# apache/incubator-predictionio

Measured on NVIDIA H100. Metric: ALS iterations/sec, higher is better.
Workload: dtype f32

## Files before the change

### incubator-predictionio_b200/csrc/als_kernels.cuh

```cuda
#pragma once
#include <cuda_runtime.h>
#include <stdint.h>

#include "als_lockstep.cuh"

namespace pio {

struct SolveParams {
  const long long* ptr;
  const int* idx;
  const float* val;
  const float* src;
  float* dst;
  const float* yty;
  const float* nreg;
  int* fail;
  float lambda;
  float alpha;
  int k;
  int row_begin;
  int row_end;
  int dst_row_offset;
  const unsigned* absmax;
  const long long* wl_beg;
// ... 501 lines not shown
    for (int o = lane; o < SLOT + KP; o += 32) {
      float s = 0.f;
      for (int q = p0; q < p1; ++q) s += p.partial[(size_t)q * (SLOT + KP) + o];
      slot[o] = s;
    }
    __syncwarp();
    chol_solve_warp<Cfg::WARP_CHOL ? KP : 16, Cfg::TB, Cfg::BLK, IMPLICIT>(
        slot, bv, p.yty, p.lambda * p.nreg[r], p.k, colbuf, dinv, p.dst + (size_t)(p.dst_row_offset + r) * KP, p.fail);
  }
}

constexpr int FIN128_WARPS = 6;
constexpr int FIN128_FLOATS = LsLayout<128>::STRIDE + 128 + 80;

template <bool IMPLICIT>
__global__ void __launch_bounds__(32 * FIN128_WARPS, 1)
als_finish_ls128_kernel(const SolveParams p, const int* __restrict__ row_part_ptr, int row0, int n_rows, int part0) {
  using LL = LsLayout<128>;
  constexpr int PF = LL::SIZE + 128;
  extern __shared__ __align__(16) float fsm128[];
  const int warp = threadIdx.x >> 5, lane = threadIdx.x & 31;
  float* slot = fsm128 + warp * FIN128_FLOATS;
  float* bv = slot + LL::STRIDE;
  float* colbuf = bv + 128;
#pragma unroll 1
  for (int base = blockIdx.x * FIN128_WARPS; base < n_rows; base += gridDim.x * FIN128_WARPS) {
    const int rr = base + warp;
    const bool have = rr < n_rows;
    const int r = row0 + (have ? rr : 0);
    if (have) {
      const int p0 = row_part_ptr[r] - part0, p1 = row_part_ptr[r + 1] - part0;
      for (int o = lane; o < PF / 4; o += 32) {
        float4 s = make_float4(0.f, 0.f, 0.f, 0.f);
        for (int q = p0; q < p1; ++q) {
          const float4 v = __ldg(reinterpret_cast<const float4*>(p.partial + (size_t)q * PF) + o);
          s.x += v.x; s.y += v.y; s.z += v.z; s.w += v.w;
        }
        if (o < LL::SIZE / 4) reinterpret_cast<float4*>(slot)[o] = s;
        else reinterpret_cast<float4*>(bv)[o - LL::SIZE / 4] = s;
      }
      if (IMPLICIT) {
        __syncwarp();
        ls_add_yty<128>(slot, p.yty);
      }
    }
    __syncthreads();
    if (have)
      chol_lockstep<128>(slot, bv, p.lambda * p.nreg[r], p.k, colbuf, p.dst + (size_t)(p.dst_row_offset + r) * 128, true,
                         p.fail);
    __syncthreads();
  }
}

constexpr int GRAM_THREADS = 256;
constexpr int GRAM_ROWS = 32;
constexpr int GRAM_GROUPS = 8;
struct GramMap {
  int cls[GRAM_GROUPS];
  int slot_of[GRAM_GROUPS];
};

template <int KP>
__global__ void __launch_bounds__(GRAM_THREADS)
gram_partial_kernel(const float* __restrict__ X, const int* __restrict__ p2i, int n_rows, double* __restrict__ partial,
                    int slot0, int bpg, const GramMap map) {
  constexpr int TM = KP / 16;
  __shared__ __align__(16) float tile[GRAM_ROWS * KP];
  const int tid = threadIdx.x, ty = tid / 16, tx = tid % 16;
  double acc[TM][TM];
#pragma unroll
  for (int i = 0; i < TM; ++i)
#pragma unroll
    for (int j = 0; j < TM; ++j) acc[i][j] = 0.0;
  const int lg = blockIdx.x / bpg, b = blockIdx.x % bpg, g = map.cls[lg];
  const int rem = n_rows % 16;
  const int T = 2 * (n_rows / 16) + (g < rem ? 1 : 0) + (15 - g < rem ? 1 : 0);
  const int per = (T + bpg - 1) / bpg;
  const int t0 = min(T, b * per);
  const int t1 = min(T, t0 + per);
  for (int base = t0; base < t1; base += GRAM_ROWS) {
    const int nr = min(GRAM_ROWS, t1 - base);
    for (int o = tid; o < GRAM_ROWS * KP / 4; o += GRAM_THREADS) {
      const int rr = o / (KP / 4);
      float4 v = make_float4(0.f, 0.f, 0.f, 0.f);
      if (rr < nr) {
        const int t = base + rr;
        const int pos = 16 * (t >> 1) + ((t & 1) ? 15 - g : g);
        v = reinterpret_cast<const float4*>(X + (size_t)__ldg(p2i + pos) * KP)[o % (KP / 4)];
      }
      reinterpret_cast<float4*>(tile)[o] = v;
    }
    __syncthreads();
#pragma unroll 4
    for (int rr = 0; rr < GRAM_ROWS; ++rr) {
      double a[TM], bb[TM];
#pragma unroll
      for (int i = 0; i < TM; ++i) {
        a[i] = (double)tile[rr * KP + ty * TM + i];
        bb[i] = (double)tile[rr * KP + tx * TM + i];
      }
#pragma unroll
      for (int i = 0; i < TM; ++i)
#pragma unroll
        for (int j = 0; j < TM; ++j) acc[i][j] = fma(a[i], bb[j], acc[i][j]);
    }
    __syncthreads();
  }
  double* out = partial + ((size_t)(slot0 + lg) * bpg + b) * KP * KP;
#pragma unroll
  for (int i = 0; i < TM; ++i)
#pragma unroll
    for (int j = 0; j < TM; ++j) out[(ty * TM + i) * KP + tx * TM + j] = acc[i][j];
}

__global__ void gram_group_kernel(const double* __restrict__ partial, int blocks_per_group, int n, int g0,
                                  double* __restrict__ gsum) {
  const int o = blockIdx.x * blockDim.x + threadIdx.x;
  const int g = g0 + blockIdx.y;
  if (o >= n) return;
  const double* p = partial + (size_t)g * blocks_per_group * n;
  double s = 0.0;
  for (int q = 0; q < blocks_per_group; ++q) s += p[(size_t)q * n + o];
  gsum[(size_t)g * n + o] = s;
}

__global__ void gram_reduce_kernel(const double* __restrict__ gsum, int n, float* __restrict__ out, const GramMap map) {
  const int o = blockIdx.x * blockDim.x + threadIdx.x;
  if (o >= n) return;
  double s = 0.0;
#pragma unroll
  for (int g = 0; g < GRAM_GROUPS; ++g) s += gsum[(size_t)map.slot_of[g] * n + o];
  out[o] = (float)s;
}

}
```

### incubator-predictionio_b200/csrc/pio_als.cu

```cuda
#include "../../include/pio_als.h"

#include <cuda_runtime.h>
#include <dlfcn.h>
#include <math.h>
#include <nccl.h>
#include <stdarg.h>
#include <stdio.h>
#include <stdlib.h>
#include <string.h>

#include <chrono>
#include <algorithm>
#include <array>
#include <deque>
#include <exception>
#include <map>
#include <memory>
#include <mutex>
#include <string>
#include <type_traits>
#include <vector>

#include "als_kernels.cuh"
#include "als_mma_kernel.cuh"
// ... 312 lines not shown
    int tz = h3 == 0 ? 64 : __ffsll((long long)h3) - 1;
    if (tz > 9) tz = 9;
    r[e] = (float)(1 + tz);
  } else {
    r[e] = (float)(1 + (int)(h3 % 5ull));
  }
}

struct Side {
  int n = 0;
  int R = 0;
  int n_internal = 0;
  int bits = 1;
  int* perm = nullptr;
  int* inv = nullptr;
  int* rpos = nullptr;
  int* p2i = nullptr;
  uint32_t* deg = nullptr;
  uint32_t* npos = nullptr;
  long long* ptr = nullptr;
  int* idx = nullptr;
  float* val = nullptr;
  long long nnz_local = 0;
  float* nreg = nullptr;
  float* F = nullptr;
  int* cand_ext = nullptr;
  int n_active = 0, n_heavy = 0;
  SidePlan plan;
  long long* part_beg = nullptr;
  long long* part_end = nullptr;
  int* row_part_ptr = nullptr;
  float* partial = nullptr;
  int n_parts = 0;
  std::vector<int> h_row_part_ptr;
};

enum EvKind { EV_SOLVE = 0, EV_GRAM = 1, EV_COMM = 2, EV_SOLVE_USER = 3, EV_NKIND = 4 };
struct EvPair {
  cudaEvent_t a, b;
  int kind;
};

}

using namespace pio;

struct pio_als_handle {
  pio_als_config cfg;
  int KP = 0;
  cudaStream_t stream = nullptr;
  Side U, I;
  float* yty = nullptr;
  double* gram_partial = nullptr;
  double* gram_gsum = nullptr;
  const Side* gram_side = nullptr;
  cudaEvent_t ev_gram = nullptr;
  int gram_blocks = 0;
  int* d_fail = nullptr;
  int* d_counts = nullptr;
  unsigned* d_absmax = nullptr;
  long long* d_timing = nullptr;
  float* d_dbg = nullptr;
  size_t dbg_rows = 0;
  SolveSwitches sw;
  cudaStream_t aux = nullptr, comm_st = nullptr;
  cudaEvent_t ev_start = nullptr, ev_heavy = nullptr, ev_piece[8] = {}, ev_comm = nullptr;
  bool pieces_done = false;
  bool trace_on = false;
  std::chrono::steady_clock::time_point t_prev;
  unsigned char* srv_dev = nullptr;
  size_t srv_dev_cap = 0;
  unsigned char* srv_host = nullptr;
  unsigned char* srv_host_dev = nullptr;
  size_t srv_host_cap = 0;
  unsigned* srv_counter = nullptr;
  unsigned srv_seq = 0;
  bool serve_fused = true;
  bool score_blocked = true;
  bool serve_trace = false;
  float* tc_out = nullptr;
  size_t tc_out_rows = 0;
  bool have_ratings = false, have_init = false, trained = false;
  ncclComm_t comm = nullptr;
  std::string err;
  pio_als_stats st{};
  double phase_ms[8] = {0, 0, 0, 0, 0, 0, 0, 0};
  std::deque<EvPair> ev_pool;
  size_t ev_used = 0;
  std::mutex mu;
  int sm_count = 0;
};

namespace pio {

static int vfail(std::string& sink, int code, const char* fmt, va_list ap) {
  char buf[512];
  vsnprintf(buf, sizeof buf, fmt, ap);
  sink = buf;
  return code;
}
static int fail(pio_als_handle* h, int code, const char* fmt, ...) {
  va_list ap;
  va_start(ap, fmt);
  const int rc = vfail(h ? h->err : g_create_error, code, fmt, ap);
  va_end(ap);
  return rc;
// ... 704 lines not shown
            tp.sp = p;
            tp.out = h->sw.tc_split ? h->tc_out : nullptr;
            tp.out_row0 = L.row_begin;
            rc = solve_launch(h, tc::Api::kernel(imp), L.grid, tc::Api::kThreads, tc::Api::kSmem, false, st, tp);
            break;
          default:
            rc = fp32();
        }
        break;
      case STAGE_TC_SOLVE:
        rc = solve_launch(h, tc::Api::solver(imp), L.grid, 32 * tc::Api::kSolveWarps, tc::Api::kSolveSmem, false, st, p,
                          (const float*)h->tc_out, L.row_begin);
        break;
    }
    if (rc) return rc;
    record_events((int)i + 1);
  }
  if (pair) {
    cudaStreamWaitEvent(h->stream, h->ev_heavy, 0);
    h->pieces_done = true;
  }
  return PIO_ALS_OK;
}

static int launch_solve(pio_als_handle* h, Side& dst, const Side& src) {
  switch (h->KP) {
    case 16: return launch_solve_cfg<Cfg16>(h, dst, src);
    case 32: return launch_solve_cfg<Cfg32>(h, dst, src);
    case 64: return launch_solve_cfg<Cfg64>(h, dst, src);
    default: return launch_solve_cfg<Cfg128>(h, dst, src);
  }
}

static bool gram_sharded(const pio_als_handle* h) { return h->cfg.world_size > 1 && GRAM_GROUPS % h->cfg.world_size == 0; }
static void gram_layout(const pio_als_handle* h, GramMap& m, int& my_groups, int& slot0) {
  const bool shard = gram_sharded(h);
  const int W = shard ? h->cfg.world_size : 1, me = shard ? h->cfg.world_rank : 0;
  my_groups = GRAM_GROUPS / W;
  slot0 = me * my_groups;
  int seen[GRAM_GROUPS] = {}, mine = 0;
  for (int g = 0; g < GRAM_GROUPS; ++g) {
    const int blk = g / W, pos = g % W;
    const int owner = (blk & 1) ? (W - 1 - pos) : pos;
    m.slot_of[g] = owner * my_groups + seen[owner]++;
    if (owner == me) m.cls[mine++] = g;
  }
  for (int lg = mine; lg < GRAM_GROUPS; ++lg) m.cls[lg] = 0;
}
static int gram_local(pio_als_handle* h, const Side& s) {
  GramMap m;
  int my_groups, slot0;
  gram_layout(h, m, my_groups, slot0);
  const int bpg = h->gram_blocks / GRAM_GROUPS, n = h->KP * h->KP, grid = my_groups * bpg;
  switch (h->KP) {
    case 16: gram_partial_kernel<16><<<grid, GRAM_THREADS, 0, h->stream>>>(s.F, s.p2i, s.n, h->gram_partial, slot0, bpg, m); break;
    case 32: gram_partial_kernel<32><<<grid, GRAM_THREADS, 0, h->stream>>>(s.F, s.p2i, s.n, h->gram_partial, slot0, bpg, m); break;
    case 64: gram_partial_kernel<64><<<grid, GRAM_THREADS, 0, h->stream>>>(s.F, s.p2i, s.n, h->gram_partial, slot0, bpg, m); break;
    default: gram_partial_kernel<128><<<grid, GRAM_THREADS, 0, h->stream>>>(s.F, s.p2i, s.n, h->gram_partial, slot0, bpg, m); break;
  }
  LAUNCHED(h);
  gram_group_kernel<<<dim3(nblk(n, 128), my_groups), 128, 0, h->stream>>>(h->gram_partial, bpg, n, slot0, h->gram_gsum);
  LAUNCHED(h);
  CK(h, cudaGetLastError());
  return PIO_ALS_OK;
}
static int gram_exchange(pio_als_handle* h, cudaStream_t comm_stream) {
  if (!gram_sharded(h)) return PIO_ALS_OK;
  const int n = h->KP * h->KP, my_groups = GRAM_GROUPS / h->cfg.world_size;
  const size_t cnt = (size_t)my_groups * n;
  if (nccl_api().AllGather(h->gram_gsum + (size_t)h->cfg.world_rank * cnt, h->gram_gsum, cnt, ncclDouble, h->comm, comm_stream) !=
      ncclSuccess)
    return fail(h, PIO_ALS_ERR_COMM, "ncclAllGather (YtY class sums) failed");
  return PIO_ALS_OK;
}
static int gram_reduce(pio_als_handle* h, const Side& s) {
  GramMap m;
  int my_groups, slot0;
  gram_layout(h, m, my_groups, slot0);
  const int n = h->KP * h->KP;
  gram_reduce_kernel<<<nblk(n, 256), 256, 0, h->stream>>>(h->gram_gsum, n, h->yty, m);
  LAUNCHED(h);
  CK(h, cudaGetLastError());
  h->gram_side = &s;
  return PIO_ALS_OK;
}

static int half_step(pio_als_handle* h, Side& dst, const Side& src, bool more) {
  cudaStream_t st = h->stream;
  const bool implicit = h->cfg.implicit_prefs != 0;
  if (implicit && h->gram_side != &src) {
    const EvPair e = next_ev(h, EV_GRAM);
    cudaEventRecord(e.a, st);
    int grc = gram_local(h, src);
    if (!grc) grc = gram_exchange(h, st);
    if (!grc) grc = gram_reduce(h, src);
    if (grc) return grc;
    cudaEventRecord(e.b, st);
  }
  {
    const EvPair e = next_ev(h, &dst == &h->U ? EV_SOLVE_USER : EV_SOLVE);
    cudaEventRecord(e.a, st);
    h->pieces_done = false;
    if (h->gram_side == &dst) h->gram_side = nullptr;
    if (dst.plan.kernel == SOLVE_PAIR) {
      const long long n = (long long)src.n_internal * h->KP;
      CK(h, cudaMemsetAsync(h->d_absmax, 0, sizeof(unsigned), st));
      pr::abs_max_kernel<<<4 * h->sm_count, 256, 0, st>>>(src.F, n, h->d_absmax);
      LAUNCHED(h);
    }
    const int rc = launch_solve(h, dst, src);
    if (rc) return rc;
    cudaEventRecord(e.b, st);
  }
  const bool prep = implicit && more;
  bool gram_pending = false;
  if (h->cfg.world_size > 1) {
    NcclApi& nc = nccl_api();
    const int W = h->cfg.world_size, me = h->cfg.world_rank;
    const EvPair e = next_ev(h, EV_COMM);
    if (h->pieces_done && h->sw.n_pieces > 1) {
      cudaStream_t sc = h->comm_st;
      const int C = h->sw.n_pieces;
      bool first = true;
      for (int c = 0; c < C; ++c) {
        const long long lo = (long long)dst.R * c / C, hi = (long long)dst.R * (c + 1) / C;
        if (hi <= lo) continue;
        cudaStreamWaitEvent(sc, h->ev_piece[c], 0);
        if (lo < dst.n_heavy) cudaStreamWaitEvent(sc, h->ev_heavy, 0);
        if (first) { cudaEventRecord(e.a, st); first = false; }
        const size_t cnt = (size_t)(hi - lo) * h->KP;
        if (nc.GroupStart() != ncclSuccess) return fail(h, PIO_ALS_ERR_COMM, "ncclGroupStart failed");
        for (int p = 0; p < W; ++p) {
          if (p == me) continue;
          if (nc.Send(dst.F + ((size_t)me * dst.R + lo) * h->KP, cnt, ncclFloat, p, h->comm, sc) != ncclSuccess ||
              nc.Recv(dst.F + ((size_t)p * dst.R + lo) * h->KP, cnt, ncclFloat, p, h->comm, sc) != ncclSuccess)
            return fail(h, PIO_ALS_ERR_COMM, "ncclSend/ncclRecv (factor pieces) failed");
        }
        if (nc.GroupEnd() != ncclSuccess) return fail(h, PIO_ALS_ERR_COMM, "ncclGroupEnd failed");
      }
      if (prep && gram_sharded(h)) {
        if (dst.n_heavy > 0) cudaStreamWaitEvent(st, h->ev_heavy, 0);
        const EvPair g = next_ev(h, EV_GRAM);
        cudaEventRecord(g.a, st);
        const int grc = gram_local(h, dst);
        if (grc) return grc;
        cudaEventRecord(g.b, st);
        cudaEventRecord(h->ev_gram, st);
        cudaStreamWaitEvent(sc, h->ev_gram, 0);
        const int xrc = gram_exchange(h, sc);
        if (xrc) return xrc;
        gram_pending = true;
      }
      cudaEventRecord(e.b, sc);
      cudaEventRecord(h->ev_comm, sc);
      cudaStreamWaitEvent(st, h->ev_comm, 0);
    } else {
      cudaEventRecord(e.a, st);
// ... 40 lines not shown
  NcclApi& a = nccl_api();
  if (!a.ok) return fail(nullptr, PIO_ALS_ERR_COMM, "libnccl.so.2 not loadable");
  ncclUniqueId id;
  if (a.GetUniqueId(&id) != ncclSuccess) return fail(nullptr, PIO_ALS_ERR_COMM, "ncclGetUniqueId failed");
  static_assert(sizeof(ncclUniqueId) == 128, "ncclUniqueId size");
  memcpy(out_id, &id, 128);
  return PIO_ALS_OK;
}

const char* pio_als_last_error(const pio_als_handle* h) { return h ? h->err.c_str() : g_create_error.c_str(); }

static int create_common(pio_als_handle* h) {
  int ndev = 0;
  cudaError_t ce = cudaGetDeviceCount(&ndev);
  if (ce != cudaSuccess || ndev == 0)
    return fail(nullptr, PIO_ALS_ERR_CUDA, "no CUDA device available (%s); this library has no CPU fallback",
                cudaGetErrorString(ce));
  if (h->cfg.device < 0 || h->cfg.device >= ndev) return fail(nullptr, PIO_ALS_ERR_ARG, "bad device %d", h->cfg.device);
  cudaDeviceProp pr;
  if (cudaGetDeviceProperties(&pr, h->cfg.device) != cudaSuccess) return fail(nullptr, PIO_ALS_ERR_CUDA, "cudaGetDeviceProperties");
  if (pr.major != 9 || pr.minor != 0)
    return fail(nullptr, PIO_ALS_ERR_CUDA, "device %d is sm_%d%d; this library is built for sm_90a (H100) only",
                h->cfg.device, pr.major, pr.minor);
  h->sm_count = pr.multiProcessorCount;
  h->st.sm_count = pr.multiProcessorCount;
  if (cudaSetDevice(h->cfg.device) != cudaSuccess) return fail(nullptr, PIO_ALS_ERR_CUDA, "cudaSetDevice");
  if (cudaStreamCreateWithFlags(&h->stream, cudaStreamNonBlocking) != cudaSuccess)
    return fail(nullptr, PIO_ALS_ERR_CUDA, "cudaStreamCreate");
  cudaMemPool_t pool;
  if (cudaDeviceGetDefaultMemPool(&pool, h->cfg.device) == cudaSuccess) {
    uint64_t thr = UINT64_MAX;
    cudaMemPoolSetAttribute(pool, cudaMemPoolAttrReleaseThreshold, &thr);
  }
  h->KP = pad_rank(h->cfg.rank);
  int prio_lo = 0, prio_hi = 0;
  cudaDeviceGetStreamPriorityRange(&prio_lo, &prio_hi);
  if (cudaStreamCreateWithFlags(&h->aux, cudaStreamNonBlocking) != cudaSuccess ||
      cudaStreamCreateWithPriority(&h->comm_st, cudaStreamNonBlocking, prio_hi) != cudaSuccess)
    return fail(nullptr, PIO_ALS_ERR_CUDA, "cudaStreamCreate");
  {
    cudaEvent_t* evs[5] = {&h->ev_start, &h->ev_heavy, &h->ev_comm, &h->ev_gram, nullptr};
    for (int i = 0; evs[i]; ++i)
      if (cudaEventCreateWithFlags(evs[i], cudaEventDisableTiming) != cudaSuccess) return fail(nullptr, PIO_ALS_ERR_CUDA, "cudaEventCreate");
    for (int i = 0; i < 8; ++i)
      if (cudaEventCreateWithFlags(&h->ev_piece[i], cudaEventDisableTiming) != cudaSuccess) return fail(nullptr, PIO_ALS_ERR_CUDA, "cudaEventCreate");
    if (const char* v = getenv("PIO_ALS_SERVE_FUSED")) h->serve_fused = atoi(v) != 0;
    if (const char* v = getenv("PIO_ALS_SERVE_TRACE")) h->serve_trace = atoi(v) != 0;
    if (const char* v = getenv("PIO_ALS_SCORE_BLOCKED")) h->score_blocked = atoi(v) != 0;
  }
  h->sw = read_solve_switches(getenv, h->KP, h->cfg.world_size);
  h->gram_blocks = GRAM_GROUPS * h->sm_count;
  if (cudaMallocAsync((void**)&h->yty, sizeof(float) * h->KP * h->KP, h->stream) != cudaSuccess ||
      cudaMallocAsync((void**)&h->gram_partial, sizeof(double) * (size_t)h->gram_blocks * h->KP * h->KP, h->stream) != cudaSuccess ||
      cudaMallocAsync((void**)&h->gram_gsum, sizeof(double) * (size_t)GRAM_GROUPS * h->KP * h->KP, h->stream) != cudaSuccess ||
      cudaMallocAsync((void**)&h->d_fail, sizeof(int), h->stream) != cudaSuccess ||
      cudaMallocAsync((void**)&h->d_counts, 4 * sizeof(int), h->stream) != cudaSuccess ||
      cudaMallocAsync((void**)&h->d_absmax, 2 * sizeof(unsigned), h->stream) != cudaSuccess)
    return fail(nullptr, PIO_ALS_ERR_CUDA, "device allocation failed");
  cudaMemsetAsync(h->yty, 0, sizeof(float) * h->KP * h->KP, h->stream);
  cudaMemsetAsync(h->d_fail, 0, sizeof(int), h->stream);
  return PIO_ALS_OK;
}

int pio_als_create(const pio_als_config* cfg, pio_als_handle** out) {
  if (!cfg || !out) return fail(nullptr, PIO_ALS_ERR_ARG, "null argument");
  *out = nullptr;
  if (cfg->abi_version != PIO_ALS_ABI_VERSION) return fail(nullptr, PIO_ALS_ERR_ARG, "abi_version mismatch");
  if (cfg->rank < 1 || cfg->rank > 128) return fail(nullptr, PIO_ALS_ERR_ARG, "rank must be in 1..128 (got %d)", cfg->rank);
  if (cfg->n_users < 1 || cfg->n_items < 1) return fail(nullptr, PIO_ALS_ERR_ARG, "n_users and n_items must be >= 1");
  if (cfg->world_size < 1 || cfg->world_rank < 0 || cfg->world_rank >= cfg->world_size)
    return fail(nullptr, PIO_ALS_ERR_ARG, "bad world_size/world_rank");
  if (!(cfg->lambda >= 0.0)) return fail(nullptr, PIO_ALS_ERR_ARG, "lambda must be >= 0");
  pio_als_handle* h = new pio_als_handle();
  h->cfg = *cfg;
  int rc = create_common(h);
  if (rc == PIO_ALS_OK && cfg->world_size > 1) {
    NcclApi& a = nccl_api();
    if (!a.ok) rc = fail(nullptr, PIO_ALS_ERR_COMM, "libnccl.so.2 not loadable");
    else {
      ncclUniqueId id;
      memcpy(&id, cfg->nccl_id, 128);
      ncclResult_t r = a.CommInitRank(&h->comm, cfg->world_size, id, cfg->world_rank);
      if (r != ncclSuccess) rc = fail(nullptr, PIO_ALS_ERR_COMM, "ncclCommInitRank failed: %s", a.GetErrorString ? a.GetErrorString(r) : "?");
    }
  }
  if (rc != PIO_ALS_OK) {
    pio_als_destroy(h);
    return rc;
  }
  *out = h;
  return PIO_ALS_OK;
}

void pio_als_destroy(pio_als_handle* h) {
  if (!h) return;
  if (h->stream) {
    cudaSetDevice(h->cfg.device);
    free_side(h, h->U, false);
    free_side(h, h->I, false);
    dfree(h, h->yty);
    dfree(h, h->gram_partial);
    dfree(h, h->gram_gsum);
    dfree(h, h->d_fail);
    dfree(h, h->d_counts);
    dfree(h, h->d_absmax);
    cudaStreamSynchronize(h->stream);
    if (h->tc_out) cudaFree(h->tc_out);
    if (h->d_dbg) cudaFree(h->d_dbg);
    if (h->d_timing) cudaFree(h->d_timing);
    for (auto& e : h->ev_pool) {
      cudaEventDestroy(e.a);
      cudaEventDestroy(e.b);
    }
    if (h->comm) nccl_api().CommDestroy(h->comm);
    if (h->ev_start) cudaEventDestroy(h->ev_start);
    if (h->ev_heavy) cudaEventDestroy(h->ev_heavy);
    if (h->ev_comm) cudaEventDestroy(h->ev_comm);
    if (h->ev_gram) cudaEventDestroy(h->ev_gram);
    for (int i = 0; i < 8; ++i)
      if (h->ev_piece[i]) cudaEventDestroy(h->ev_piece[i]);
    if (h->srv_dev) cudaFree(h->srv_dev);
    if (h->srv_host) cudaFreeHost(h->srv_host);
    if (h->srv_counter) cudaFree(h->srv_counter);
    if (h->aux) cudaStreamDestroy(h->aux);
    if (h->comm_st) cudaStreamDestroy(h->comm_st);
    cudaStreamDestroy(h->stream);
  }
  delete h;
}

static int set_ratings_impl(pio_als_handle* h, const int32_t* user, const int32_t* item, const float* rating, int64_t nnz,
                            int dedup_mode, const int64_t* ts, bool on_device, bool sharded) {
  if (!h) return PIO_ALS_ERR_ARG;
  const bool may_be_empty = sharded && h->cfg.world_size > 1;
  if (nnz < 0 || (nnz == 0 && !may_be_empty))
    return fail(h, PIO_ALS_ERR_ARG, "ratings cannot be empty (the templates require(!ratings.take(1).isEmpty))");
  if (nnz > 0 && (!user || !item || !rating)) return fail(h, PIO_ALS_ERR_ARG, "null rating arrays");
  if (nnz >= (1ll << 32)) return fail(h, PIO_ALS_ERR_ARG, "nnz must be < 2^32 per call");
  if (dedup_mode < 0 || dedup_mode > 2) return fail(h, PIO_ALS_ERR_ARG, "bad dedup_mode %d", dedup_mode);
  std::lock_guard<std::mutex> lk(h->mu);
  CK(h, cudaSetDevice(h->cfg.device));
  cudaStream_t st = h->stream;
  cudaEvent_t a, b;
  cudaEventCreate(&a);
  cudaEventCreate(&b);
  cudaEventRecord(a, st);
  int rc;
  {
    Scratch tmp(h->stream);
    const int *du = user, *di = item;
    const float* dr = rating;
    const long long* dts = (const long long*)ts;
    auto stage = [&]() -> int {
      if (on_device || nnz == 0) return PIO_ALS_OK;
// ... 1268 lines not shown
  }
  const size_t nu = hd.n_users, ni = hd.n_items, k = hd.rank;
  const long long expect = (long long)sizeof hd + (long long)(nu + ni) + (long long)sizeof(float) * (long long)((nu + ni) * k);
  if (fseek(f, 0, SEEK_END) != 0 || ftell(f) != expect || fseek(f, (long)sizeof hd, SEEK_SET) != 0) {
    fclose(f);
    return fail(nullptr, PIO_ALS_ERR_IO, "%s is truncated or has trailing bytes (expected %lld bytes)", path, expect);
  }
  try {
    std::vector<float> uf(nu * k), itf(ni * k);
    std::vector<uint8_t> uh(nu), ih(ni);
    bool ok = fread(uh.data(), 1, nu, f) == nu && fread(ih.data(), 1, ni, f) == ni &&
              fread(uf.data(), sizeof(float), nu * k, f) == nu * k && fread(itf.data(), sizeof(float), ni * k, f) == ni * k;
    fclose(f);
    f = nullptr;
    if (!ok) return fail(nullptr, PIO_ALS_ERR_IO, "%s is truncated", path);
    pio_als_config cfg{};
    cfg.abi_version = PIO_ALS_ABI_VERSION;
    cfg.rank = hd.rank;
    cfg.implicit_prefs = hd.implicit_prefs;
    cfg.n_users = hd.n_users;
    cfg.n_items = hd.n_items;
    cfg.device = device;
    cfg.world_size = 1;
    cfg.lambda = hd.lambda;
    cfg.alpha = hd.alpha;
    return pio_als_model_import(&cfg, uf.data(), itf.data(), uh.data(), ih.data(), out);
  } catch (const std::exception& e) {
    if (f) fclose(f);
    return fail(nullptr, PIO_ALS_ERR_IO, "pio_als_load: %s", e.what());
  }
}

__attribute__((visibility("default"))) int pio_als_debug_dump(pio_als_handle* h, float* out, long long n_floats) {
  if (!h || !h->d_dbg) return PIO_ALS_ERR_STATE;
  cudaStreamSynchronize(h->stream);
  size_t n = h->dbg_rows * (tc::ASLOT + tc::KP);
  if ((size_t)n_floats < n) n = (size_t)n_floats;
  return cudaMemcpy(out, h->d_dbg, n * sizeof(float), cudaMemcpyDeviceToHost) == cudaSuccess ? PIO_ALS_OK : PIO_ALS_ERR_CUDA;
}

__attribute__((visibility("default"))) int pio_als_debug_timing(pio_als_handle* h, long long* out, long long n) {
  if (!h || !h->d_timing) return PIO_ALS_ERR_STATE;
  cudaStreamSynchronize(h->stream);
  size_t m = (size_t)h->sm_count * 16 * 8;
  if ((size_t)n < m) m = (size_t)n;
  return cudaMemcpy(out, h->d_timing, m * sizeof(long long), cudaMemcpyDeviceToHost) == cudaSuccess ? PIO_ALS_OK : PIO_ALS_ERR_CUDA;
}

#define CK0(call)                                                                                         \
  do {                                                                                                    \
    cudaError_t e_ = (call);                                                                              \
    if (e_ != cudaSuccess) return fail(nullptr, PIO_ALS_ERR_CUDA, "%s failed: %s", #call, cudaGetErrorString(e_)); \
  } while (0)

#define EVF(call)                          \
  do {                                     \
    const int rc_ = (call);                \
    if (rc_ != PIO_ALS_OK) return rc_;     \
  } while (0)

extern "C++" {
template <int N>
__global__ void __launch_bounds__(32) lockstep_probe_kernel(const float* __restrict__ A, const float* __restrict__ b, int n,
                                                            float ridge, float* __restrict__ x, int reps, int* fail) {
  using LL = LsLayout<N>;
  constexpr int LANES = N / 4, NM = 32 / LANES;
  extern __shared__ __align__(16) float sm[];
  float* bvec = sm + NM * LL::STRIDE;
  float* colbuf = bvec + NM * 80 + (N > 64 ? N : 0);
  const int lane = threadIdx.x & 31, grp = lane / LANES;
  for (int base = blockIdx.x * NM; base < n; base += gridDim.x * NM) {
    for (int rep = 0; rep < reps; ++rep) {
      for (int m = 0; m < NM; ++m) {
        const int mi = base + m;
        float* slot = sm + m * LL::STRIDE;
        for (int o = lane; o < N * N; o += 32) {
          const int r = o / N, c = o % N;
          if (c <= r) slot[LL::at(r, c)] = mi < n ? A[(size_t)mi * N * N + o] : (r == c ? 1.f : 0.f);
        }
        for (int o = lane; o < N; o += 32) bvec[m * (N > 64 ? N : 80) + o] = mi < n ? b[(size_t)mi * N + o] : 0.f;
      }
      __syncwarp();
      const int mine = base + grp;
      chol_lockstep<N>(sm + grp * LL::STRIDE, bvec + grp * (N > 64 ? N : 80), ridge, N, colbuf + grp * 80,
                       x + (size_t)(mine < n ? mine : 0) * N, mine < n, fail);
      __syncwarp();
    }
  }
}
}

__attribute__((visibility("default"))) int pio_als_debug_lockstep(int device, int N, int n, const float* A, const float* b,
                                                                  float ridge, float* x, int reps, float* ms_out,
                                                                  int* fail_out) {
  if ((N != 64 && N != 128) || n < 1 || !A || !b || !x) return PIO_ALS_ERR_ARG;
  CK0(cudaSetDevice(device));
  CallMem tmp(0);
  float *dA = nullptr, *db = nullptr, *dx = nullptr;
  int* dfail = nullptr;
  CK0(tmp.device(&dA, (size_t)n * N * N));
  CK0(tmp.device(&db, (size_t)n * N));
  CK0(tmp.device(&dx, (size_t)n * N));
  CK0(tmp.device(&dfail, 1));
  CK0(cudaMemset(dfail, 0, sizeof(int)));
  CK0(cudaMemcpy(dA, A, sizeof(float) * (size_t)n * N * N, cudaMemcpyHostToDevice));
  CK0(cudaMemcpy(db, b, sizeof(float) * (size_t)n * N, cudaMemcpyHostToDevice));
// ... 3411 lines not shown
```

### incubator-predictionio_b200/native.py

```python
from __future__ import annotations

import ctypes as C
import os
import subprocess
from dataclasses import dataclass, field
from pathlib import Path
from typing import Any, Dict, List, Optional, Sequence

import numpy as np

PKG_DIR = Path(__file__).resolve().parent
REPO_ROOT = PKG_DIR.parent
LIB_PATH = PKG_DIR / "libpio_als.so"
CSRC = PKG_DIR / "csrc"

ABI_VERSION = 2
DEDUP_NONE, DEDUP_SUM, DEDUP_KEEP_LAST = 0, 1, 2
INIT_CALLER, INIT_HASH = 0, 1
SIM_KEEP_QUERY_ITEMS = 1
ERR_ARG, ERR_CUDA, ERR_STATE, ERR_NUMERIC, ERR_IO, ERR_COMM, ERR_NOMEM = -1, -2, -3, -4, -5, -6, -7

EXPORTED_SYMBOLS = [
    "pio_als_abi_version", "pio_als_device_count", "pio_als_nccl_unique_id", "pio_als_create",
    "pio_als_destroy", "pio_als_last_error", "pio_als_set_ratings_coo", "pio_als_set_ratings_coo_device", "pio_als_set_ratings_coo_sharded",
# ... 375 lines not shown
        nu = 0 if uf is None else uf.shape[0]
        cfg = Config()
        cfg.abi_version, cfg.rank, cfg.implicit_prefs = ABI_VERSION, int(k), int(bool(implicit))
        cfg.n_users, cfg.n_items, cfg.device, cfg.world_size = int(nu), int(ni), int(device), 1
        cfg.lambda_, cfg.alpha = float(lam), float(alpha)
        uh = None if user_has is None else np.ascontiguousarray(user_has, np.uint8)
        ih = None if item_has is None else np.ascontiguousarray(item_has, np.uint8)
        h = C.c_void_p()
        _check(lib().pio_als_model_import(C.byref(cfg), _ptr(uf, C.c_float), _ptr(itf, C.c_float), _ptr(uh, C.c_uint8),
                                          _ptr(ih, C.c_uint8), C.byref(h)))
        return cls(rank=int(k), n_users=max(int(nu), 1), n_items=int(ni), _handle=h)

    def stats(self) -> dict:
        st = Stats()
        self._check(lib().pio_als_get_stats(self._h, C.byref(st)))
        out = {name: getattr(st, name) for name, _ in Stats._fields_}
        out["last_score_path"] = {name for name, bit in SCORE_PATH_BITS.items() if st.last_score_path & bit}
        return out

    _SIDE_SCALARS = ("n", "R", "n_internal", "bits", "nnz_local", "n_active", "n_heavy", "n_parts", "nnz", "heavy_t",
                     "part_len")

    def debug_side(self, side: str) -> dict:
        f = lib().pio_als_debug_side
        sc = np.zeros(len(self._SIDE_SCALARS), np.int64)
        which = {"user": 0, "item": 1}[side]
        nul = [None] * 12
        self._check(f(self._h, C.c_int(which), _ptr(sc, C.c_int64), *nul))
        out = dict(zip(self._SIDE_SCALARS, (int(x) for x in sc)))
        n, R, nl = out["n"], out["R"], out["nnz_local"]
        arrs = dict(deg=np.empty(n, np.uint32), npos=np.empty(n, np.uint32), perm=np.empty(n, np.int32),
                    inv=np.empty(out["n_internal"], np.int32), rpos=np.empty(n, np.int32), ptr=np.empty(R + 1, np.int64),
                    idx=np.empty(nl, np.int32), val=np.empty(nl, np.float32), nreg=np.empty(R, np.float32),
                    part_beg=np.empty(out["n_parts"], np.int64), part_end=np.empty(out["n_parts"], np.int64),
                    row_part_ptr=np.zeros(out["n_heavy"] + 1, np.int32))
        self._check(f(self._h, C.c_int(which), _ptr(sc, C.c_int64), *(C.c_void_p(a.ctypes.data) for a in arrs.values())))
        out.update(arrs)
        return out

    def phase_ms(self) -> dict:
        out = (C.c_double * 8)()
        self._check(lib().pio_als_get_phase_ms(self._h, out))
        return {"item_solve_ms": out[0], "user_solve_ms": out[1], "gram_ms": out[2], "comm_ms": out[3],
                "item_kernel": _KERNEL_NAMES[int(out[4])], "user_kernel": _KERNEL_NAMES[int(out[5])],
                "iterations": int(out[6])}


def synth_ratings_device(device, n_users, n_items, nnz, seed, implicit, start, d_user, d_item, d_rating):
    _check(lib().pio_als_synth_ratings_device(C.c_int(device), C.c_int32(n_users), C.c_int32(n_items), C.c_int64(nnz),
                                              C.c_int64(seed), C.c_int(int(implicit)), C.c_int64(start),
                                              C.c_void_p(d_user), C.c_void_p(d_item), C.c_void_p(d_rating)))


def ids_encode(strings, device=0):
    if isinstance(strings, tuple):
        buf, off = strings
        buf = np.ascontiguousarray(buf, np.uint8)
        off = np.ascontiguousarray(off, np.int64)
    else:
        buf, off = _str_column([s if isinstance(s, (bytes, bytearray)) else str(s).encode("utf-8") for s in strings])
    n = off.shape[0] - 1
    idx = np.empty(n, np.int32)
    first = np.empty(max(n, 1), np.int64)
    nu = C.c_int32(0)
    _check(lib().pio_ids_encode(C.c_int(device), _ptr(buf, C.c_uint8) if buf.size else None, _ptr(off, C.c_int64),
                                C.c_int64(n), _ptr(idx, C.c_int32), _ptr(first, C.c_int64), C.byref(nu)))
    return idx, first[:nu.value]


class EvalFolds:

    def __init__(self, user, item, rating, k_fold: int, device: int = 0):
        self._h = C.c_void_p()
        user = np.ascontiguousarray(user, np.int32)
        item = np.ascontiguousarray(item, np.int32)
        rating = np.ascontiguousarray(rating, np.float64)
        if not (user.shape == item.shape == rating.shape) or user.ndim != 1:
            raise ValueError("user/item/rating must be 1-D arrays of equal length")
        self.k_fold, self.device = int(k_fold), int(device)
        _check(lib().pio_eval_folds_create(C.c_int(device), _ptr(user, C.c_int32), _ptr(item, C.c_int32),
                                           _ptr(rating, C.c_double), C.c_int64(user.shape[0]), C.c_int32(k_fold),
                                           C.byref(self._h)))

    def close(self):
        if self._h:
            lib().pio_eval_folds_destroy(self._h)
            self._h = C.c_void_p()

    def __del__(self):
        try:
            self.close()
        except Exception:
            pass

    def sizes(self, fold: int) -> tuple:
        out = np.zeros(4, np.int64)
        _check(lib().pio_eval_folds_sizes(self._h, C.c_int32(fold), _ptr(out, C.c_int64)))
        return tuple(int(x) for x in out)

    def maps(self, fold: int) -> dict:
        nu, ni, _, nq = self.sizes(fold)
        out = {"user": np.empty(nu, np.int32), "item": np.empty(ni, np.int32), "query_user": np.empty(nq, np.int32),
               "query_train_user": np.empty(nq, np.int32)}
        _check(lib().pio_eval_folds_maps(self._h, C.c_int32(fold), *_addrs(out, "user", "item", "query_user",
                                                                           "query_train_user")))
        return out
# ... 641 lines not shown
```

Measured before the change: 35.27.

## Restructure YtY gram kernel: triangular warp tiles, cp.async double buffer, fused absmax

```diff
diff --git a/incubator-predictionio_b200/csrc/als_kernels.cuh b/incubator-predictionio_b200/csrc/als_kernels.cuh
--- a/incubator-predictionio_b200/csrc/als_kernels.cuh
+++ b/incubator-predictionio_b200/csrc/als_kernels.cuh
@@ -577,8 +577,6 @@
   }
 }
 
-constexpr int GRAM_THREADS = 256;
-constexpr int GRAM_ROWS = 32;
 constexpr int GRAM_GROUPS = 8;
 struct GramMap {
   int cls[GRAM_GROUPS];
@@ -586,75 +584,154 @@
 };
 
 template <int KP>
-__global__ void __launch_bounds__(GRAM_THREADS)
+struct GramGeom {
+  static constexpr int NB = KP / 16 * (KP / 16 + 1) / 2;
+  static constexpr int BPW = NB > 16 ? 2 : 1;
+  static constexpr int WARPS = NB / BPW;
+  static constexpr int THREADS = 32 * WARPS;
+  static constexpr int MIN_CTAS = KP == 128 ? 1 : 3;
+  static constexpr int ROWS = KP == 128 ? 16 : 32;
+  static constexpr int LD = ROWS * KP / 4;
+  static constexpr int NLD = (LD + THREADS - 1) / THREADS;
+};
+static_assert(GramGeom<128>::NB % GramGeom<128>::BPW == 0, "YtY blocks per warp");
+
+template <int KP>
+__global__ void __launch_bounds__(GramGeom<KP>::THREADS, GramGeom<KP>::MIN_CTAS)
 gram_partial_kernel(const float* __restrict__ X, const int* __restrict__ p2i, int n_rows, double* __restrict__ partial,
-                    int slot0, int bpg, const GramMap map) {
-  constexpr int TM = KP / 16;
-  __shared__ __align__(16) float tile[GRAM_ROWS * KP];
-  const int tid = threadIdx.x, ty = tid / 16, tx = tid % 16;
-  double acc[TM][TM];
-#pragma unroll
-  for (int i = 0; i < TM; ++i)
-#pragma unroll
-    for (int j = 0; j < TM; ++j) acc[i][j] = 0.0;
-  const int lg = blockIdx.x / bpg, b = blockIdx.x % bpg, g = map.cls[lg];
+                    float* __restrict__ bmax, int slot0, int bpg, const GramMap map) {
+  using G = GramGeom<KP>;
+  __shared__ __align__(16) double tile[G::ROWS * KP];
+  __shared__ __align__(16) float stage[2][G::ROWS * KP];
+  __shared__ float wmax[G::WARPS];
+  const int tid = threadIdx.x, warp = tid >> 5, lane = tid & 31, ry = lane >> 3, cx = lane & 7;
+  int bi[G::BPW], bj[G::BPW];
+#pragma unroll
+  for (int w = 0; w < G::BPW; ++w) {
+    const int q = warp + w * G::WARPS;
+    int I = 0;
+    while ((I + 1) * (I + 2) / 2 <= q) ++I;
+    bi[w] = I;
+    bj[w] = q - I * (I + 1) / 2;
+  }
+  double acc[G::BPW][4][2];
+#pragma unroll
+  for (int w = 0; w < G::BPW; ++w)
+#pragma unroll
+    for (int i = 0; i < 4; ++i) acc[w][i][0] = acc[w][i][1] = 0.0;
+  float m = 0.f;
+  const int lg = blockIdx.x / bpg, b = blockIdx.x % bpg;
+  int g = 0;
+#pragma unroll
+  for (int i = 0; i < GRAM_GROUPS; ++i) g = i == lg ? map.cls[i] : g;
   const int rem = n_rows % 16;
   const int T = 2 * (n_rows / 16) + (g < rem ? 1 : 0) + (15 - g < rem ? 1 : 0);
   const int per = (T + bpg - 1) / bpg;
   const int t0 = min(T, b * per);
   const int t1 = min(T, t0 + per);
-  for (int base = t0; base < t1; base += GRAM_ROWS) {
-    const int nr = min(GRAM_ROWS, t1 - base);
-    for (int o = tid; o < GRAM_ROWS * KP / 4; o += GRAM_THREADS) {
-      const int rr = o / (KP / 4);
-      float4 v = make_float4(0.f, 0.f, 0.f, 0.f);
-      if (rr < nr) {
-        const int t = base + rr;
-        const int pos = 16 * (t >> 1) + ((t & 1) ? 15 - g : g);
-        v = reinterpret_cast<const float4*>(X + (size_t)__ldg(p2i + pos) * KP)[o % (KP / 4)];
-      }
-      reinterpret_cast<float4*>(tile)[o] = v;
-    }
+  int idx[G::NLD];
+  auto row_ids = [&](int base) {
+#pragma unroll
+    for (int j = 0; j < G::NLD; ++j) {
+      const int o = tid + j * G::THREADS, t = base + o / (KP / 4);
+      idx[j] = -1;
+      if (o < G::LD && t < t1) idx[j] = __ldg(p2i + 16 * (t >> 1) + ((t & 1) ? 15 - g : g));
+    }
+  };
+  auto copy = [&](float* dst) {
+#pragma unroll
+    for (int j = 0; j < G::NLD; ++j) {
+      const int o = tid + j * G::THREADS;
+      if (idx[j] >= 0) cp_async16(dst + 4 * o, X + (size_t)idx[j] * KP + 4 * (o % (KP / 4)));
+    }
+    cp_async_commit();
+  };
+  row_ids(t0);
+  copy(stage[0]);
+  row_ids(t0 + G::ROWS);
+  int k = 0;
+  for (int base = t0; base < t1; base += G::ROWS, ++k) {
+    const int nr = min(G::ROWS, t1 - base);
+    copy(stage[(k + 1) & 1]);
+    row_ids(base + 2 * G::ROWS);
+    cp_async_wait<1>();
     __syncthreads();
-#pragma unroll 4
-    for (int rr = 0; rr < GRAM_ROWS; ++rr) {
-      double a[TM], bb[TM];
-#pragma unroll
-      for (int i = 0; i < TM; ++i) {
-        a[i] = (double)tile[rr * KP + ty * TM + i];
-        bb[i] = (double)tile[rr * KP + tx * TM + i];
-      }
-#pragma unroll
-      for (int i = 0; i < TM; ++i)
-#pragma unroll
-        for (int j = 0; j < TM; ++j) acc[i][j] = fma(a[i], bb[j], acc[i][j]);
+    const float2* src = reinterpret_cast<const float2*>(stage[k & 1]);
+    for (int o = tid; o < nr * KP / 2; o += G::THREADS) {
+      const float2 v = src[o];
+      m = fmaxf(m, fmaxf(fabsf(v.x), fabsf(v.y)));
+      reinterpret_cast<double2*>(tile)[o] = make_double2(v.x, v.y);
     }
     __syncthreads();
-  }
+#pragma unroll 2
+    for (int rr = 0; rr < nr; ++rr) {
+      const double2* row = reinterpret_cast<const double2*>(tile + rr * KP);
+#pragma unroll
+      for (int w = 0; w < G::BPW; ++w) {
+        const double2 a0 = row[8 * bi[w] + ry], a1 = row[8 * bi[w] + 4 + ry], c = row[8 * bj[w] + cx];
+        const double a[4] = {a0.x, a0.y, a1.x, a1.y};
+#pragma unroll
+        for (int i = 0; i < 4; ++i) {
+          acc[w][i][0] = fma(a[i], c.x, acc[w][i][0]);
+          acc[w][i][1] = fma(a[i], c.y, acc[w][i][1]);
+        }
+      }
+    }
+  }
+  cp_async_wait<0>();
   double* out = partial + ((size_t)(slot0 + lg) * bpg + b) * KP * KP;
 #pragma unroll
-  for (int i = 0; i < TM; ++i)
-#pragma unroll
-    for (int j = 0; j < TM; ++j) out[(ty * TM + i) * KP + tx * TM + j] = acc[i][j];
-}
-
-__global__ void gram_group_kernel(const double* __restrict__ partial, int blocks_per_group, int n, int g0,
-                                  double* __restrict__ gsum) {
-  const int o = blockIdx.x * blockDim.x + threadIdx.x;
+  for (int w = 0; w < G::BPW; ++w)
+#pragma unroll
+    for (int i = 0; i < 4; ++i) {
+      const int r = 16 * bi[w] + 2 * ry + (i & 1) + (i >> 1) * 8;
+      reinterpret_cast<double2*>(out + (size_t)r * KP + 16 * bj[w])[cx] = make_double2(acc[w][i][0], acc[w][i][1]);
+    }
+#pragma unroll
+  for (int o = 16; o > 0; o >>= 1) m = fmaxf(m, __shfl_xor_sync(0xffffffffu, m, o));
+  if (lane == 0) wmax[warp] = m;
+  __syncthreads();
+  if (tid == 0) {
+    float v = 0.f;
+    for (int w = 0; w < G::WARPS; ++w) v = fmaxf(v, wmax[w]);
+    bmax[(slot0 + lg) * bpg + b] = v;
+  }
+}
+
+__global__ void gram_group_kernel(const double* __restrict__ partial, const float* __restrict__ bmax, int blocks_per_group,
+                                  int kp, int g0, double* __restrict__ gsum) {
+  const int n = kp * kp, o = blockIdx.x * blockDim.x + threadIdx.x;
   const int g = g0 + blockIdx.y;
-  if (o >= n) return;
+  double* out = gsum + (size_t)g * (n + 1);
+  if (o == n) {
+    float v = 0.f;
+    for (int q = 0; q < blocks_per_group; ++q) v = fmaxf(v, bmax[g * blocks_per_group + q]);
+    out[n] = v;
+    return;
+  }
+  const int r = o / kp, c = o % kp;
+  if (o > n || r < c) return;
   const double* p = partial + (size_t)g * blocks_per_group * n;
   double s = 0.0;
+#pragma unroll 8
   for (int q = 0; q < blocks_per_group; ++q) s += p[(size_t)q * n + o];
-  gsum[(size_t)g * n + o] = s;
-}
-
-__global__ void gram_reduce_kernel(const double* __restrict__ gsum, int n, float* __restrict__ out, const GramMap map) {
+  out[o] = s;
+  out[c * kp + r] = s;
+}
+
+__global__ void gram_reduce_kernel(const double* __restrict__ gsum, int n, float* __restrict__ out,
+                                   unsigned* __restrict__ absmax, const GramMap map) {
   const int o = blockIdx.x * blockDim.x + threadIdx.x;
-  if (o >= n) return;
+  if (o > n) return;
   double s = 0.0;
-#pragma unroll
-  for (int g = 0; g < GRAM_GROUPS; ++g) s += gsum[(size_t)map.slot_of[g] * n + o];
+  if (o == n) {
+#pragma unroll
+    for (int g = 0; g < GRAM_GROUPS; ++g) s = fmax(s, gsum[(size_t)map.slot_of[g] * (n + 1) + n]);
+    *absmax = __float_as_uint((float)s);
+    return;
+  }
+#pragma unroll
+  for (int g = 0; g < GRAM_GROUPS; ++g) s += gsum[(size_t)map.slot_of[g] * (n + 1) + o];
   out[o] = (float)s;
 }
 
diff --git a/incubator-predictionio_b200/csrc/pio_als.cu b/incubator-predictionio_b200/csrc/pio_als.cu
--- a/incubator-predictionio_b200/csrc/pio_als.cu
+++ b/incubator-predictionio_b200/csrc/pio_als.cu
@@ -388,6 +388,7 @@
   Side U, I;
   float* yty = nullptr;
   double* gram_partial = nullptr;
+  float* gram_bmax = nullptr;
   double* gram_gsum = nullptr;
   const Side* gram_side = nullptr;
   cudaEvent_t ev_gram = nullptr;
@@ -1198,14 +1199,18 @@
   int my_groups, slot0;
   gram_layout(h, m, my_groups, slot0);
   const int bpg = h->gram_blocks / GRAM_GROUPS, n = h->KP * h->KP, grid = my_groups * bpg;
+  auto partial = [&](auto kernel, int threads) {
+    kernel<<<grid, threads, 0, h->stream>>>(s.F, s.p2i, s.n, h->gram_partial, h->gram_bmax, slot0, bpg, m);
+  };
   switch (h->KP) {
-    case 16: gram_partial_kernel<16><<<grid, GRAM_THREADS, 0, h->stream>>>(s.F, s.p2i, s.n, h->gram_partial, slot0, bpg, m); break;
-    case 32: gram_partial_kernel<32><<<grid, GRAM_THREADS, 0, h->stream>>>(s.F, s.p2i, s.n, h->gram_partial, slot0, bpg, m); break;
-    case 64: gram_partial_kernel<64><<<grid, GRAM_THREADS, 0, h->stream>>>(s.F, s.p2i, s.n, h->gram_partial, slot0, bpg, m); break;
-    default: gram_partial_kernel<128><<<grid, GRAM_THREADS, 0, h->stream>>>(s.F, s.p2i, s.n, h->gram_partial, slot0, bpg, m); break;
+    case 16: partial(gram_partial_kernel<16>, GramGeom<16>::THREADS); break;
+    case 32: partial(gram_partial_kernel<32>, GramGeom<32>::THREADS); break;
+    case 64: partial(gram_partial_kernel<64>, GramGeom<64>::THREADS); break;
+    default: partial(gram_partial_kernel<128>, GramGeom<128>::THREADS); break;
   }
   LAUNCHED(h);
-  gram_group_kernel<<<dim3(nblk(n, 128), my_groups), 128, 0, h->stream>>>(h->gram_partial, bpg, n, slot0, h->gram_gsum);
+  gram_group_kernel<<<dim3(nblk(n + 1, 128), my_groups), 128, 0, h->stream>>>(h->gram_partial, h->gram_bmax, bpg, h->KP,
+                                                                              slot0, h->gram_gsum);
   LAUNCHED(h);
   CK(h, cudaGetLastError());
   return PIO_ALS_OK;
@@ -1213,7 +1218,7 @@
 static int gram_exchange(pio_als_handle* h, cudaStream_t comm_stream) {
   if (!gram_sharded(h)) return PIO_ALS_OK;
   const int n = h->KP * h->KP, my_groups = GRAM_GROUPS / h->cfg.world_size;
-  const size_t cnt = (size_t)my_groups * n;
+  const size_t cnt = (size_t)my_groups * (n + 1);
   if (nccl_api().AllGather(h->gram_gsum + (size_t)h->cfg.world_rank * cnt, h->gram_gsum, cnt, ncclDouble, h->comm, comm_stream) !=
       ncclSuccess)
     return fail(h, PIO_ALS_ERR_COMM, "ncclAllGather (YtY class sums) failed");
@@ -1224,7 +1229,7 @@
   int my_groups, slot0;
   gram_layout(h, m, my_groups, slot0);
   const int n = h->KP * h->KP;
-  gram_reduce_kernel<<<nblk(n, 256), 256, 0, h->stream>>>(h->gram_gsum, n, h->yty, m);
+  gram_reduce_kernel<<<nblk(n + 1, 256), 256, 0, h->stream>>>(h->gram_gsum, n, h->yty, h->d_absmax, m);
   LAUNCHED(h);
   CK(h, cudaGetLastError());
   h->gram_side = &s;
@@ -1248,7 +1253,7 @@
     cudaEventRecord(e.a, st);
     h->pieces_done = false;
     if (h->gram_side == &dst) h->gram_side = nullptr;
-    if (dst.plan.kernel == SOLVE_PAIR) {
+    if (dst.plan.kernel == SOLVE_PAIR && !implicit) {
       const long long n = (long long)src.n_internal * h->KP;
       CK(h, cudaMemsetAsync(h->d_absmax, 0, sizeof(unsigned), st));
       pr::abs_max_kernel<<<4 * h->sm_count, 256, 0, st>>>(src.F, n, h->d_absmax);
@@ -1395,7 +1400,8 @@
   h->gram_blocks = GRAM_GROUPS * h->sm_count;
   if (cudaMallocAsync((void**)&h->yty, sizeof(float) * h->KP * h->KP, h->stream) != cudaSuccess ||
       cudaMallocAsync((void**)&h->gram_partial, sizeof(double) * (size_t)h->gram_blocks * h->KP * h->KP, h->stream) != cudaSuccess ||
-      cudaMallocAsync((void**)&h->gram_gsum, sizeof(double) * (size_t)GRAM_GROUPS * h->KP * h->KP, h->stream) != cudaSuccess ||
+      cudaMallocAsync((void**)&h->gram_bmax, sizeof(float) * (size_t)h->gram_blocks, h->stream) != cudaSuccess ||
+      cudaMallocAsync((void**)&h->gram_gsum, sizeof(double) * (size_t)GRAM_GROUPS * (h->KP * h->KP + 1), h->stream) != cudaSuccess ||
       cudaMallocAsync((void**)&h->d_fail, sizeof(int), h->stream) != cudaSuccess ||
       cudaMallocAsync((void**)&h->d_counts, 4 * sizeof(int), h->stream) != cudaSuccess ||
       cudaMallocAsync((void**)&h->d_absmax, 2 * sizeof(unsigned), h->stream) != cudaSuccess)
@@ -1443,6 +1449,7 @@
     free_side(h, h->I, false);
     dfree(h, h->yty);
     dfree(h, h->gram_partial);
+    dfree(h, h->gram_bmax);
     dfree(h, h->gram_gsum);
     dfree(h, h->d_fail);
     dfree(h, h->d_counts);
@@ -2817,6 +2824,59 @@
     cudaError_t e_ = (call);                                                                              \
     if (e_ != cudaSuccess) return fail(nullptr, PIO_ALS_ERR_CUDA, "%s failed: %s", #call, cudaGetErrorString(e_)); \
   } while (0)
+
+__attribute__((visibility("default"))) int pio_als_debug_gram(int device, const float* x, int32_t n, int32_t rank,
+                                                              int32_t blocks_per_class, int32_t reps, float* yty_out,
+                                                              uint32_t* absmax_out, float* ms_out) {
+  if (!x || !yty_out || !absmax_out || n < 1 || rank < 1 || rank > 128) return fail(nullptr, PIO_ALS_ERR_ARG, "bad argument");
+  if (cudaSetDevice(device) != cudaSuccess) return fail(nullptr, PIO_ALS_ERR_CUDA, "cudaSetDevice(%d) failed", device);
+  pio_als_handle h;
+  h.cfg.world_size = 1;
+  h.cfg.world_rank = 0;
+  h.KP = pad_rank(rank);
+  const int KP = h.KP;
+  if (cudaDeviceGetAttribute(&h.sm_count, cudaDevAttrMultiProcessorCount, device) != cudaSuccess)
+    return fail(nullptr, PIO_ALS_ERR_CUDA, "cudaDeviceGetAttribute");
+  h.gram_blocks = GRAM_GROUPS * (blocks_per_class > 0 ? blocks_per_class : h.sm_count);
+  CallMem tmp;
+  CK0(tmp.stream(&h.stream));
+  Side s;
+  s.n = n;
+  std::vector<int> ident(n);
+  for (int i = 0; i < n; ++i) ident[i] = i;
+  CK0(tmp.device(&s.F, (size_t)n * KP));
+  CK0(tmp.device(&s.p2i, (size_t)n));
+  CK0(tmp.device(&h.yty, (size_t)KP * KP));
+  CK0(tmp.device(&h.gram_partial, (size_t)h.gram_blocks * KP * KP));
+  CK0(tmp.device(&h.gram_bmax, (size_t)h.gram_blocks));
+  CK0(tmp.device(&h.gram_gsum, (size_t)GRAM_GROUPS * (KP * KP + 1)));
+  CK0(tmp.device(&h.d_absmax, (size_t)1));
+  CK0(cudaMemsetAsync(s.F, 0, sizeof(float) * (size_t)n * KP, h.stream));
+  CK0(cudaMemcpy2DAsync(s.F, sizeof(float) * KP, x, sizeof(float) * rank, sizeof(float) * rank, n, cudaMemcpyHostToDevice,
+                        h.stream));
+  CK0(cudaMemcpyAsync(s.p2i, ident.data(), sizeof(int) * (size_t)n, cudaMemcpyHostToDevice, h.stream));
+  cudaEvent_t e0 = nullptr, e1 = nullptr;
+  CK0(tmp.event(&e0));
+  CK0(tmp.event(&e1));
+  int rc = PIO_ALS_OK;
+  for (int r = 0; r <= reps && !rc; ++r) {
+    if (r == 1) cudaEventRecord(e0, h.stream);
+    rc = gram_local(&h, s);
+    if (!rc) rc = gram_reduce(&h, s);
+  }
+  cudaEventRecord(e1, h.stream);
+  if (!rc && cudaMemcpyAsync(yty_out, h.yty, sizeof(float) * KP * KP, cudaMemcpyDeviceToHost, h.stream) != cudaSuccess) rc = PIO_ALS_ERR_CUDA;
+  if (!rc && cudaMemcpyAsync(absmax_out, h.d_absmax, sizeof(unsigned), cudaMemcpyDeviceToHost, h.stream) != cudaSuccess) rc = PIO_ALS_ERR_CUDA;
+  const cudaError_t se = cudaStreamSynchronize(h.stream);
+  if (!rc && se != cudaSuccess) rc = fail(nullptr, PIO_ALS_ERR_CUDA, "YtY pass: %s", cudaGetErrorString(se));
+  if (!rc && reps > 0 && ms_out) {
+    cudaEventElapsedTime(ms_out, e0, e1);
+    *ms_out /= reps;
+  }
+  if (rc && !h.err.empty()) g_create_error = h.err;
+  return rc;
+}
+
 
 #define EVF(call)                          \
   do {                                     \
diff --git a/incubator-predictionio_b200/native.py b/incubator-predictionio_b200/native.py
--- a/incubator-predictionio_b200/native.py
+++ b/incubator-predictionio_b200/native.py
@@ -451,6 +451,18 @@
                                               C.c_void_p(d_user), C.c_void_p(d_item), C.c_void_p(d_rating)))
 
 
+def gram_debug(x, blocks_per_class=0, reps=0, device=0):
+    x = np.ascontiguousarray(x, np.float32)
+    n, rank = x.shape
+    kp = 16 if rank <= 16 else 32 if rank <= 32 else 64 if rank <= 64 else 128
+    yty = np.empty((kp, kp), np.float32)
+    bits, ms = C.c_uint32(0), C.c_float(0.0)
+    f = lib().pio_als_debug_gram
+    f.argtypes = [C.c_int, C.c_void_p, C.c_int32, C.c_int32, C.c_int32, C.c_int32, C.c_void_p, C.c_void_p, C.c_void_p]
+    _check(f(device, _addr(x), n, rank, blocks_per_class, reps, _addr(yty), C.addressof(bits), C.addressof(ms)))
+    return yty, bits.value, (ms.value if reps > 0 else None)
+
+
 def ids_encode(strings, device=0):
     if isinstance(strings, tuple):
         buf, off = strings
```

Result: faster. 35.82, median of 6 (+1.6%).
